# alessiodevoto/peekvit

Measured on AMD Instinct MI355X. Metric: images/sec ViT-B/16 fwd @ batch 2048, 224x224, higher is better.
Workload: dtype f16; 1 GPU; vit_b_16 forward, batch 2048/GPU, 224x224; global_batch=2048, parallelism=replicas x1 (batch-sharded, no collective), precision_mode=auto, streams=1, operands=IEEE fp16 operands, fp32 accumulate (same MFMA rate as bf16), range-guarded, range_guard_fallbacks=0

## Files before the change

peekvit_amd/_build.py:

```python
from __future__ import annotations

import glob
import os
import subprocess
import sys

HERE = os.path.dirname(os.path.abspath(__file__))
CSRC = os.path.join(HERE, "csrc")
LIB = os.path.join(HERE, "libpeekvit_hip.so")
LIB_F16 = os.path.join(HERE, "libpeekvit_hip_f16.so")
HIPCC = os.environ.get("HIPCC", "/opt/rocm/bin/hipcc")
FLAGS = ["--offload-arch=gfx950", "-O3", "-std=c++17", "-fPIC", "-Wno-unused-result"]
HEADERS = ("peekvit_hip.h", "peekvit_hip_moe.h", "peekvit_hip_ee.h", "peekvit_hip_sparse.h", "peekvit_hip_pct.h")
FILE_FLAGS = {"pv_attention.hip": ["-mllvm", "-amdgpu-mfma-vgpr-form=1"], "pv_rowops.hip": ["-fno-slp-vectorize"],
              "pv_ee.hip": ["-fno-slp-vectorize"],
              "pv_sparse.hip": ["-fno-slp-vectorize"],
              "pv_pct.hip": ["-fno-slp-vectorize"]}


def sources():
    return sorted(glob.glob(os.path.join(CSRC, "*.hip")))


def _stale() -> bool:
    if not os.path.exists(LIB) or not os.path.exists(LIB_F16):
        return True
    t = min(os.path.getmtime(LIB), os.path.getmtime(LIB_F16))
    deps = sources() + glob.glob(os.path.join(CSRC, "*.h")) + [os.path.join(os.path.dirname(HERE), "include", h) for h in HEADERS] + [os.path.abspath(__file__)]
    return any(os.path.getmtime(d) > t for d in deps)


def build(force: bool = False, verbose: bool = False) -> str:
    if not force and not _stale():
        return LIB
    procs = []
    variants = [("build", [], LIB), ("build_f16", ["-DPV_OPERAND_F16"], LIB_F16)]
    objs = {lib: [] for _, _, lib in variants}
    for sub, defs, lib in variants:
        objdir = os.path.join(HERE, sub)
        os.makedirs(objdir, exist_ok=True)
        for src in sources():
            obj = os.path.join(objdir, os.path.basename(src)[:-4] + ".o")
            objs[lib].append(obj)
            cmd = [HIPCC, *FLAGS, *FILE_FLAGS.get(os.path.basename(src), []), *defs, "-c", src, "-o", obj]
            if verbose:
                print(" ".join(cmd))
            procs.append((src, subprocess.Popen(cmd, stdout=subprocess.PIPE, stderr=subprocess.STDOUT)))
    for src, p in procs:
        out, _ = p.communicate()
        if p.returncode != 0:
# ... 35 lines not shown
```

peekvit_amd/_lib.py:

```python
from __future__ import annotations

import ctypes as C
import os
import threading

import torch

from ._build import LIB

_i64, _f32, _p, _i32 = C.c_int64, C.c_float, C.c_void_p, C.c_int32

PV_EPI_BIAS_BF16, PV_EPI_BIAS_GELU_BF16, PV_EPI_BIAS_RES_F32, PV_EPI_BIAS_POS_F32 = 0, 1, 2, 3
PV_EPI_BIAS_F32, PV_EPI_BIAS_GELU_SPLIT_BF16 = 4, 5
PV_EPI_BIAS_GELU_PAIR_BF16, PV_EPI_GELU_GRAD_BF16 = 6, 7
PV_WS_TRANSPOSE_COLSUM, PV_WS_COLSUM, PV_WS_LAYERNORM_BWD, PV_WS_GEMM_COLSUM_PARTIAL, PV_WS_GEMM_SPLITK = 1, 2, 3, 4, 5


class GemmArgs(C.Structure):
    _fields_ = [("struct_size", C.c_uint64), ("A", _p), ("W", _p), ("bias", _p), ("out", _p), ("res", _p), ("row_scale", _p), ("pos", _p),
                ("M", _i64), ("N", _i64), ("K", _i64), ("lda", _i64), ("ldw", _i64), ("ldo", _i64), ("ldr", _i64),
                ("rows_per_img_in", _i64), ("rows_per_img_out", _i64), ("row_off", _i64), ("qcols", _i64),
                ("qscale", _f32), ("epilogue", _i32),
                ("ln_gamma", _p), ("ln_beta", _p), ("ln_row_scale", _p), ("ln_out", _p), ("ln_eps", _f32),
                ("ksplit", _i32), ("colsum_partial", _p),
# ... 58 lines not shown
    "pv_residual_gate_bwd": (C.c_int, [_p, _p, _p, _p, _p, _p, _p, _f32, _f32, _p, _p, _p, _p, _i64, _i64, _i64, _p]),
    "pv_attention_varlen_bf16": (C.c_int, [_p, _p, _p, _p, _i64, _i64, _i64, _i64, _p, _p]),
    "pv_act_step": (C.c_int, [_p, _p, _p, _p, _i64, _i64, _i64, _p, _p, _p, _p, _p, _p, _i64, _p, _f32, _f32, _f32, C.c_int,
                              _p, _p, _p, _p, _p, _p, _p]),
}

SIGNATURES_MOE = {
    "pv_moe_packed_rows": (C.c_int64, [_i64, _i64]),
    "pv_moe_route_scratch_size": (C.c_int64, [_i64, _i64]),
    "pv_moe_route": (C.c_int, [_p, _i64, _i64, _i64, _p, _p, _f32, _p, _p, _i64, _p, _p, _p, _p, _p, _p, _p, _p, _i64, _p]),
    "pv_gemm_grouped_bf16": (C.c_int, [C.POINTER(GemmArgs), _p, _i64, _i64, _i64, _p, _i64, _p]),
    "pv_moe_gather_bf16": (C.c_int, [_p, _i64, _i64, _p, _p, _i64, _i64, _i64, _i64, _p, _p]),
}

SIGNATURES_EE = {
    "pv_exit_head_f32": (C.c_int, [_p, _i64, _p, _p, _f32, _p, _p, _p, _i64, _i64, _i64, _p]),
    "pv_exit_step": (C.c_int, [_p, _i64, _p, _i64, _i64, _f32, _i64, _p, _p, _i64, _p, _p, _i64, _p, _p, _p, _p]),
    "pv_gather_images_f32": (C.c_int, [_p, _i64, _p, _i64, _i64, _p, _p]),
}

SIGNATURES_SPARSE = {
    "pv_attention_varlen_w_bf16": (C.c_int, [_p, _p, _p, _p, _i64, _i64, _i64, _i64, _p, _p]),
    "pv_residual_pack_step": (C.c_int, [_p, _p, _p, _p, _i64, _i64, _i64, _p, _p, _p, _p, _f32, _f32, _p,
                                        _p, _p, _p, _p, _p, _p, _p, _p, _p, _p, _p, _f32, _p, _p]),
}

SIGNATURES_PCT = {
    "pv_arpe_embed": (C.c_int, [_p, _p, _p, _p, _p, _p, _p, _p, _p, _p, _p, _i64, _i64, _i64, _i64, _i64, _i64, _p]),
    "pv_layernorm_f32_bf16": (C.c_int, [_p, _i64, _p, _p, _p, _p, _i64, _i64, _i64, _f32, _p]),
    "pv_mean_pool_f32": (C.c_int, [_p, _p, _i64, _i64, _i64, _p]),
    "pv_pct_head_f32": (C.c_int, [_p, _p, _p, _p, _p, _p, _p, _p, _i64, _i64, _i64, _i64, _p]),
}

ABI_VERSION = 10
_lock = threading.Lock()
_libs: dict = {}

_OPERAND_DEFAULT = "bf16"
_tls = threading.local()
LIB_F16 = os.path.join(os.path.dirname(os.path.abspath(__file__)), "libpeekvit_hip_f16.so")


def current_operand() -> str:
    return getattr(_tls, "operand", _OPERAND_DEFAULT)


def set_operand(op: str) -> str:
    old = current_operand()
    _tls.operand = op
    return old


def __getattr__(name):
    if name == "OPERAND":
        return current_operand()
    raise AttributeError(f"module {__name__!r} has no attribute {name!r}")


def operand_dtype():
    import torch as _t
    return _t.float16 if current_operand() == "f16" else _t.bfloat16


class PeekvitHipError(RuntimeError):
    pass


def lib_path(operand: str = "bf16") -> str:
    return LIB_F16 if operand == "f16" else LIB


def load(operand=None):
    op = current_operand() if operand is None else operand
    lib = _libs.get(op)
    if lib is not None:
        return lib
    with _lock:
        lib = _libs.get(op)
        if lib is not None:
            return lib
        path = lib_path(op)
        if not os.path.exists(path):
            raise PeekvitHipError(
                f"{path} not found: the MI355X kernels are not built. Run `python -m peekvit_amd._build` "
                "(or __graft_entry__.build()); there is no fallback path.")
        lib = C.CDLL(path)
        for name, (res, args) in {**SIGNATURES, **SIGNATURES_MOE, **SIGNATURES_EE, **SIGNATURES_SPARSE, **SIGNATURES_PCT}.items():
            fn = getattr(lib, name)
            fn.restype, fn.argtypes = res, args
        if lib.pv_version() != ABI_VERSION:
            raise PeekvitHipError(f"{path} has ABI v{lib.pv_version()}, this package binds v{ABI_VERSION}: rebuild (python -m peekvit_amd._build)")
        if lib.pv_gemm_args_size() != C.sizeof(GemmArgs):
            raise PeekvitHipError(f"{path}: pv_gemm_args is {lib.pv_gemm_args_size()} bytes in the library, {C.sizeof(GemmArgs)} in this binding")
        if lib.pv_operand_type() != (1 if op == "f16" else 0):
            raise PeekvitHipError(f"{path} was built for a different operand type")
        _libs[op] = lib
    return lib


def check(code: int, what: str = "") -> None:
    if code != 0:
        msg = load().pv_error_string(code).decode()
        raise PeekvitHipError(f"{what}: {msg} (code {code})" if what else f"{msg} (code {code})")
```

peekvit_amd/autograph.py:

```python
from __future__ import annotations

import os
import threading
from typing import Optional

import torch
import torch.nn as nn

ENABLED = os.environ.get("PEEKVIT_AMD_AUTO_GRAPH", "1") != "0"
WARM = int(os.environ.get("PEEKVIT_AMD_AUTO_GRAPH_WARM", "4"))
MAX_GRAPHS = 4
HOST_MS_BASE, HOST_MS_PER_LAYER = 0.12, 0.115
SMALL_TFLOPS = 300.0

replays = 0
captures = 0
drops = 0

_structure_epoch = 0


def _bump(*_a, **_k):
    global _structure_epoch
    _structure_epoch += 1
    return None


try:
    import torch.nn.modules.module as _m
    _m.register_module_module_registration_hook(_bump)
    _m.register_module_parameter_registration_hook(_bump)
    _m.register_module_buffer_registration_hook(_bump)
except (ImportError, AttributeError):
    ENABLED = False


def _knobs():
    from . import engine, ops
    return (engine._STREAMS, engine.LOCAL_FALLBACK, engine.SELFCHECK_IMAGES, engine.SELFCHECK_LIMIT, engine.RANK_STRICT, engine._FUSE_LN, engine._FULLROW_LN,
            engine._FOLD_LN, engine._FUSE_RANK_NORM, engine._SMALL_M_SPLITK, engine._LAST_BLOCK_ROWS, engine._GATE_NO_MASKED, engine.FALLBACK_MODE,
            engine.RANK_REPAIR, engine.RANK_TIE_GAP, engine._FUSED_PATCH_EMBED,
            getattr(ops, "knob_epoch", 0))


def launch_bound(owner: nn.Module, batch: int) -> bool:
    try:
        D, L, S = int(owner.hidden_dim), len(owner.encoder.layers), int(owner.seq_length)
        Mh = int(getattr(owner, "mlp_dim", 4 * D))
    except (AttributeError, TypeError):
        return False
    flops = batch * L * (S * D * 3 * D * 2 + 2 * S * S * D * 2 + S * D * D * 2 + 2 * S * D * Mh * 2)
    return flops / (SMALL_TFLOPS * 1e12) < (HOST_MS_BASE + HOST_MS_PER_LAYER * L) * 1e-3


class _Entry:
    __slots__ = ("warm", "graph", "sig", "params", "mods", "calls", "dead")

    def __init__(self):
        self.warm, self.graph, self.sig, self.params, self.mods, self.calls, self.dead = 0, None, None, None, None, 0, False


_version_of = __import__("operator").attrgetter("_version")


def _signature(owner: nn.Module, ent: _Entry, st) -> tuple:
    from . import engine
    layers = getattr(getattr(owner, "encoder", None), "layers", ())
    return (_structure_epoch, engine._opt_generation, tuple(map(id, layers)), sum(map(_version_of, ent.params)), _knobs(),
            st.unsafe, st.no_fold, st.hybrid, st.mlp_hybrid, owner.training)


def _hooked(ent: _Entry) -> bool:
    import torch.nn.modules.module as _m
    if _m._global_forward_hooks or _m._global_forward_pre_hooks:
# ... 96 lines not shown
```

peekvit_amd/engine.py:

```python
from __future__ import annotations

import math
import os
import threading
import warnings
import weakref
from typing import Dict, Optional, Tuple

import torch
from torch import nn

from . import _lib, autograph, ops
import contextlib

from ._lib import (PV_EPI_BIAS_BF16, PV_EPI_BIAS_F32, PV_EPI_BIAS_GELU_BF16, PV_EPI_BIAS_GELU_SPLIT_BF16, PV_EPI_BIAS_POS_F32,
                   PV_EPI_BIAS_RES_F32, PeekvitHipError)

_MODE_DEFAULT = os.environ.get("PEEKVIT_AMD_PRECISION", "auto")
_MODES = ("auto", "bf16", "f16", "bf16x3")
if _MODE_DEFAULT not in _MODES:
    raise ValueError(f"PEEKVIT_AMD_PRECISION={_MODE_DEFAULT!r}: expected one of {_MODES}")
_lib._OPERAND_DEFAULT = "f16" if _MODE_DEFAULT == "f16" else "bf16"
_mode_tls = threading.local()

# ... 909 lines not shown
                 ln=(_f32(blk.ln_2.weight), _f32(blk.ln_2.bias), eps, h2, row_scale) if fuse2 else None)
        ln2_done = fuse2
    else:
        ln2_done = _residual_gemm(att, bf16_weight(mha.out_proj.weight), _f32(mha.out_proj.bias), x1.view(R, D), x.view(R, D), R,
                                  ln=(_f32(blk.ln_2.weight), _f32(blk.ln_2.bias), eps, h2))
    if mlp_hyb:
        _mlp_half_split(blk, x1, out, R, eps, row_scale)
        return out
    if not ln2_done:
        ops.layernorm_bf16(x1, _f32(blk.ln_2.weight), _f32(blk.ln_2.bias), eps, h2, row_scale)
    _act_gemm(h2, bf16_weight(blk.mlp.fc1.weight), _f32(blk.mlp.fc1.bias), g, R, gelu=True)
    fuse_next = next_ln is not None and _ln_fusable(D, M) and next_ln.normalized_shape == (D,)
    hn = workspace.get("h", (R, D), _lib.operand_dtype(), dev) if fuse_next else None
    rowsq = None
    if next_ranks and not fuse_next and _FUSE_RANK_NORM and ops.gemm_tile_rows(R, D, M, PV_EPI_BIAS_RES_F32) == 256:
        rowsq = workspace.get("rowsq", ((D + 255) // 256, R), torch.float32, dev)
    if fuse_next or rowsq is not None:
        ops.gemm(g, bf16_weight(blk.mlp.fc2.weight), _f32(blk.mlp.fc2.bias), out.view(R, D), PV_EPI_BIAS_RES_F32, M=R,
                 res=x1.view(R, D), rowsq_out=rowsq,
                 ln=(_f32(next_ln.weight), _f32(next_ln.bias), next_ln.eps, hn, None) if fuse_next else None)
    else:
        want = next_ln is not None and next_ln.normalized_shape == (D,)
        hn = workspace.get("h", (R, D), _lib.operand_dtype(), dev) if want else None
        fuse_next = _residual_gemm(g, bf16_weight(blk.mlp.fc2.weight), _f32(blk.mlp.fc2.bias), out.view(R, D), x1.view(R, D), R,
                                   ln=(_f32(next_ln.weight), _f32(next_ln.bias), next_ln.eps, hn) if want else None)
    if fuse_next:
        out._pv_ln = (hn, _ln_key(next_ln))
    if rowsq is not None:
        out._pv_rowsq = (rowsq, _tver(out))
    return out


_LAST_BLOCK_ROWS = os.environ.get("PEEKVIT_AMD_LAST_BLOCK_ROWS", "1") != "0"
_GATE_LN1 = os.environ.get("PEEKVIT_AMD_GATE_LN1", "1") != "0"
_GATE_NO_MASKED = os.environ.get("PEEKVIT_AMD_GATE_MASKED", "0") != "1"


def rows_only_ok(blk: nn.Module) -> bool:
    import torch.nn.modules.module as _m
    if not _LAST_BLOCK_ROWS or _mode() == "bf16x3" or layer_is_hybrid() or layer_mlp_is_hybrid():
        return False
    own = ("_forward_hooks", "_forward_pre_hooks", "_backward_hooks", "_backward_pre_hooks")
    glob = ("_global_forward_hooks", "_global_forward_pre_hooks", "_global_backward_hooks", "_global_backward_pre_hooks")
    return not any(getattr(blk, n, None) for n in own) and not any(getattr(_m, n, None) for n in glob)


def block_forward_rows(blk: nn.Module, x: torch.Tensor, eps: float, nq: int, row_scale: Optional[torch.Tensor] = None,
                       h1: Optional[torch.Tensor] = None) -> torch.Tensor:
    if x.dtype != torch.float32:
        x = x.float()
    fold_in, handoff = getattr(x, "_pv_fold", None), getattr(x, "_pv_ln", None)
    if fold_in is not None and fold_in[3] != _tver(x):
        fold_in = None
    if not x.is_contiguous():
        x, fold_in, handoff = x.contiguous(), None, None
    if row_scale is not None:
        fold_in, handoff = None, None
    B, S, D = x.shape
    mha = blk.self_attention.self_attention
    H = mha.num_heads
    dh = D // H
    M = blk.mlp.fc1.out_features
    dev, R, Rq, od = x.device, B * S, B * nq, _lib.operand_dtype()
    _check_ln_range(blk.ln_1)
    _check_ln_range(blk.ln_2)
    g1, b1 = _f32(blk.ln_1.weight), _f32(blk.ln_1.bias)

    kv = workspace.get("qkv", (R, 2 * D), od, dev)
    if fold_in is not None and fold_in[2] == _ln_key(blk.ln_1) and fold_in[0].shape == (R, D):
        wg, c1, c2 = _fold_weights(mha.in_proj_weight, mha.in_proj_bias, blk.ln_1)
        stat = ops.rowstat_finalize(fold_in[1], D, blk.ln_1.eps, workspace.get("fold_stat", (R, 2), torch.float32, dev))
        ops.gemm(fold_in[0], wg[D:], None, kv, PV_EPI_BIAS_BF16, M=R, fold=(stat, c1[D:], c2[D:]))
    else:
        if h1 is not None and h1.shape == (R, D):
            h = h1
        elif handoff is not None and handoff[1] == _ln_key(blk.ln_1) and handoff[0].shape == (R, D):
            h = handoff[0]
        else:
            h = workspace.get("h", (R, D), od, dev)
            ops.layernorm_bf16(x, g1, b1, eps, h, row_scale)
        ops.gemm(h, bf16_weight(mha.in_proj_weight)[D:], _f32(mha.in_proj_bias)[D:], kv, PV_EPI_BIAS_BF16, M=R)

    xq = workspace.get("rows_x", (B, nq, D), torch.float32, dev)
    xq.copy_(x[:, :nq])
    xq = xq.view(Rq, D)
    rsq = None
    if row_scale is not None:
        rsq = workspace.get("rows_rs", (B, nq), torch.float32, dev)
        rsq.copy_(row_scale.view(B, S)[:, :nq])
    hq = workspace.get("rows_h", (Rq, D), od, dev)
    ops.layernorm_bf16(xq, g1, b1, eps, hq, rsq)
    qb = workspace.get("rows_q", (Rq, D), od, dev)
    ops.gemm(hq, bf16_weight(mha.in_proj_weight)[:D], _f32(mha.in_proj_bias)[:D], qb, PV_EPI_BIAS_BF16, M=Rq, qcols=D, qscale=float(dh) ** -0.5)
    att = workspace.get("rows_att", (Rq, D), od, dev)
    ops.attention_rows(qb, kv, att, B, S, nq, H, dh)
    x1 = workspace.get("rows_x1", (Rq, D), torch.float32, dev)
    if rsq is None:
        _residual_gemm(att, bf16_weight(mha.out_proj.weight), _f32(mha.out_proj.bias), x1, xq, Rq)
    else:
        ops.gemm(att, bf16_weight(mha.out_proj.weight), _f32(mha.out_proj.bias), x1, PV_EPI_BIAS_RES_F32, M=Rq, res=xq, row_scale=rsq)
    ops.layernorm_bf16(x1, _f32(blk.ln_2.weight), _f32(blk.ln_2.bias), eps, hq, rsq)
    g = workspace.get("rows_g", (Rq, M), od, dev)
    ops.gemm(hq, bf16_weight(blk.mlp.fc1.weight), _f32(blk.mlp.fc1.bias), g, PV_EPI_BIAS_GELU_BF16, M=Rq)
    out = torch.empty((B, nq, D), dtype=torch.float32, device=dev)
    _residual_gemm(g, bf16_weight(blk.mlp.fc2.weight), _f32(blk.mlp.fc2.bias), out.view(Rq, D), x1, Rq)
    return out


def _block_forward_x3(blk: nn.Module, x: torch.Tensor, eps: float, row_scale: Optional[torch.Tensor]) -> torch.Tensor:
    x = x.float() if x.dtype != torch.float32 else x
    x = x if x.is_contiguous() else x.contiguous()
    B, S, D = x.shape
    mha = blk.self_attention.self_attention
    H = mha.num_heads
    dh = D // H
    M = blk.mlp.fc1.out_features
    dev, R = x.device, B * S
    h3 = workspace.get("h3", (R, 3 * D), _lib.operand_dtype(), dev)
    qkv32 = workspace.get("qkv32", (R, 3 * D), torch.float32, dev)
    att3 = workspace.get("att3", (R, 3 * D), _lib.operand_dtype(), dev)
    g3 = workspace.get("g3", (R, 3 * M), _lib.operand_dtype(), dev)
    x1 = workspace.get("x1", (B, S, D), torch.float32, dev)
    out = torch.empty_like(x)
    ops.layernorm_split(x, _f32(blk.ln_1.weight), _f32(blk.ln_1.bias), eps, h3, row_scale)
    ops.gemm(h3, bf16x3_weight(mha.in_proj_weight), _f32(mha.in_proj_bias), qkv32, PV_EPI_BIAS_F32, M=R, qcols=D, qscale=float(dh) ** -0.5)
    ops.attention_f32(qkv32, att3, B, S, H, dh)
    ops.gemm(att3, bf16x3_weight(mha.out_proj.weight), _f32(mha.out_proj.bias), x1.view(R, D), PV_EPI_BIAS_RES_F32, M=R,
             res=x.view(R, D), row_scale=row_scale)
# ... 722 lines not shown
```

peekvit_amd/ops.py:

```python
from __future__ import annotations

import ctypes as C
from typing import Optional

import torch

from . import _lib
from ._lib import GemmArgs, check

launch_count = 0


class KernelTimer:

    def __init__(self):
        self.records = []

    def __enter__(self):
        global _timer
        _timer = self
        return self

    def __exit__(self, *exc):
        global _timer
# ... 232 lines not shown
    N = b.shape[1]
    assert b.shape[0] == K and part.shape == (max(ksplit, 1), M, N) and part.is_contiguous()
    args = GemmArgs(A=a.data_ptr(), W=b.data_ptr(), bias=0, out=part.data_ptr(), res=0, row_scale=0, pos=0, M=M, N=N, K=K,
                    lda=a.stride(0), ldw=b.stride(0), ldo=N, ldr=0, rows_per_img_in=0, rows_per_img_out=0, row_off=0, qcols=0,
                    qscale=1.0, epilogue=_lib.PV_EPI_BIAS_F32, ln_gamma=0, ln_beta=0, ln_row_scale=0, ln_out=0, ln_eps=0.0,
                    ksplit=int(ksplit))
    with _timed("pv_gemm_tn_bf16" + tag, a.device, 2.0 * M * N * K, 2.0 * K * (M + N) + 4.0 * max(ksplit, 1) * M * N):
        check(_lib.load().pv_gemm_tn_bf16(C.byref(args), _stream(a)), "pv_gemm_tn_bf16")
    _count()
    return part


def attention(qkv: torch.Tensor, out: torch.Tensor, B: int, S: int, H: int, dh: int, lse: Optional[torch.Tensor] = None):
    with _timed("pv_attention_bf16", qkv.device, 4.0 * B * H * S * S * dh, 8.0 * B * S * H * dh):
        if lse is None:
            check(_lib.load().pv_attention_bf16(_ptr(qkv), _ptr(out), B, S, H, dh, _attn_flag(qkv.device), _stream(qkv)), "pv_attention_bf16")
        else:
            _chk(lse, torch.float32, "lse")
            if lse.numel() != B * H * S:
                raise _lib.PeekvitHipError("attention: lse must hold B * H * S values")
            check(_lib.load().pv_attention_lse_bf16(_ptr(qkv), _ptr(out), _ptr(lse), B, S, H, dh, _attn_flag(qkv.device), _stream(qkv)), "pv_attention_lse_bf16")
    _count()
    return out


def attention_bwd_lse_ok(S: int, dh: int) -> bool:
    return attention_bwd_lse_supported(S, dh) and S >= 145


def attention_bwd_lse_supported(S: int, dh: int) -> bool:
    return dh in (48, 64) and 129 <= S <= 208


def attention_rows(q: torch.Tensor, kv: torch.Tensor, out: torch.Tensor, B: int, S: int, nq: int, H: int, dh: int):
    for t, name in ((q, "q"), (kv, "kv"), (out, "out")):
        if not (t.is_cuda and t.dtype == _lib.operand_dtype() and t.dim() == 2 and t.stride(1) == 1):
            raise _lib.PeekvitHipError(f"attention_rows: {name} must be a 2-D GPU tensor of the operand type with unit column stride")
    if q.shape[0] != B * nq or out.shape[0] != B * nq or kv.shape[0] != B * S or kv.shape[1] < 2 * H * dh:
        raise _lib.PeekvitHipError("attention_rows: shape mismatch")
    with _timed("pv_attention_rows_bf16", q.device, 4.0 * B * H * nq * S * dh, 4.0 * B * S * H * dh + 4.0 * B * nq * H * dh):
        check(_lib.load().pv_attention_rows_bf16(_ptr(q), q.stride(0), _ptr(kv), kv.stride(0), _ptr(out), out.stride(0),
                                                 B, S, nq, H, dh, _attn_flag(q.device), _stream(q)), "pv_attention_rows_bf16")
    _count()
    return out


def attention_rows_bwd(q, kv, out, dout, dq, dkv, B: int, S: int, H: int, dh: int, qscale: float):
    for t, name in ((q, "q"), (kv, "kv"), (out, "out"), (dout, "dout"), (dq, "dq"), (dkv, "dkv")):
        if not (t.is_cuda and t.dtype == _lib.operand_dtype() and t.dim() == 2 and t.stride(1) == 1):
            raise _lib.PeekvitHipError(f"attention_rows_bwd: {name} must be a 2-D GPU tensor of the operand type with unit column stride")
    if any(t.shape[0] != B for t in (q, out, dout, dq)) or kv.shape[0] != B * S or dkv.shape[0] != B * S:
        raise _lib.PeekvitHipError("attention_rows_bwd: shape mismatch")
    with _timed("pv_attention_rows_bwd_bf16", q.device, 10.0 * B * H * S * dh, 2.0 * 3 * 2 * B * S * H * dh):
        check(_lib.load().pv_attention_rows_bwd_bf16(_ptr(q), q.stride(0), _ptr(kv), kv.stride(0), _ptr(out), out.stride(0), _ptr(dout), dout.stride(0),
                                                     _ptr(dq), dq.stride(0), _ptr(dkv), dkv.stride(0), B, S, 1, H, dh, float(qscale), _stream(q)),
              "pv_attention_rows_bwd_bf16")
    _count()
    return dq, dkv


def cls_pool(x: torch.Tensor, gamma, beta, eps: float, num_cls: int) -> torch.Tensor:
    B, S, D = x.shape
    pooled = torch.empty((B, D), dtype=torch.float32, device=x.device)
    with _timed("pv_cls_pool", x.device, 0.0, 0.0):
        check(_lib.load().pv_cls_pool(_ptr(x), _ptr(gamma), _ptr(beta), _ptr(pooled), B, S, D, num_cls, float(eps),
                                      _stream(x)), "pv_cls_pool")
    _count()
    return pooled


def head(pooled: torch.Tensor, w: torch.Tensor, b) -> torch.Tensor:
    B, D = pooled.shape
    Cn = w.shape[0]
    logits = torch.empty((B, Cn), dtype=torch.float32, device=pooled.device)
    with _timed("pv_head_f32", pooled.device, 2.0 * B * D * Cn, 0.0):
# ... 576 lines not shown
```

Before: 27530 images/sec.

## Fold K/V projection into CLS-row attention to skip full-token KV GEMM

For the final block where only a few query rows (CLS) are needed, the K and V projection of all tokens is no longer materialised. Instead, each query is folded into the key weights (u = q·Wk), scores are computed directly against the raw or LayerNorm-folded tokens, a softmax-weighted token average is accumulated, and the value projection is then applied once per query row. This replaces an R x 2D x D GEMM with work that scales with the number of query rows times heads, at the cost of three new kernels, fp32 scratch buffers, and hi/lo split MFMA for precision.

```diff
diff --git a/include/peekvit_hip_cls.h b/include/peekvit_hip_cls.h
--- /dev/null
+++ b/include/peekvit_hip_cls.h
@@ -0,0 +1,27 @@
+#ifndef PEEKVIT_HIP_CLS_H
+#define PEEKVIT_HIP_CLS_H
+
+#include "peekvit_hip.h"
+
+#ifdef __cplusplus
+extern "C" {
+#endif
+
+#define PV_CLS_MAX_D 768
+#define PV_CLS_MAX_ROWS 32
+
+int pv_cls_attention_built(int64_t S, int64_t D, int64_t H, int64_t dh, int64_t nq);
+
+int pv_cls_query_fold_bf16(const uint16_t* q, int64_t ldq, const uint16_t* wk, int64_t ldw, const float* c1k, const float* c2k, float* u,
+                           float* cd, int64_t rows, int64_t H, int64_t dh, void* stream);
+
+int pv_cls_token_pass_bf16(const uint16_t* tok, int64_t ldt, const float* stat, const float* u, const float* cd, float* a, float* m,
+                           int64_t B, int64_t S, int64_t D, int64_t nr, uint32_t* range_flag, void* stream);
+
+int pv_cls_value_fold_bf16(const float* a, const float* m, const uint16_t* wv, int64_t ldw, const float* c1v, const float* c2v,
+                           uint16_t* att, int64_t ldo, int64_t rows, int64_t H, int64_t dh, void* stream);
+
+#ifdef __cplusplus
+}
+#endif
+#endif
diff --git a/peekvit_amd/_build.py b/peekvit_amd/_build.py
--- a/peekvit_amd/_build.py
+++ b/peekvit_amd/_build.py
@@ -11,11 +11,12 @@
 LIB_F16 = os.path.join(HERE, "libpeekvit_hip_f16.so")
 HIPCC = os.environ.get("HIPCC", "/opt/rocm/bin/hipcc")
 FLAGS = ["--offload-arch=gfx950", "-O3", "-std=c++17", "-fPIC", "-Wno-unused-result"]
-HEADERS = ("peekvit_hip.h", "peekvit_hip_moe.h", "peekvit_hip_ee.h", "peekvit_hip_sparse.h", "peekvit_hip_pct.h")
+HEADERS = ("peekvit_hip.h", "peekvit_hip_moe.h", "peekvit_hip_ee.h", "peekvit_hip_sparse.h", "peekvit_hip_pct.h", "peekvit_hip_cls.h")
 FILE_FLAGS = {"pv_attention.hip": ["-mllvm", "-amdgpu-mfma-vgpr-form=1"], "pv_rowops.hip": ["-fno-slp-vectorize"],
               "pv_ee.hip": ["-fno-slp-vectorize"],
               "pv_sparse.hip": ["-fno-slp-vectorize"],
-              "pv_pct.hip": ["-fno-slp-vectorize"]}
+              "pv_pct.hip": ["-fno-slp-vectorize"],
+              "pv_cls_attention.hip": ["-fno-slp-vectorize"]}
 
 
 def sources():
diff --git a/peekvit_amd/_lib.py b/peekvit_amd/_lib.py
--- a/peekvit_amd/_lib.py
+++ b/peekvit_amd/_lib.py
@@ -114,6 +114,13 @@
     "pv_pct_head_f32": (C.c_int, [_p, _p, _p, _p, _p, _p, _p, _p, _i64, _i64, _i64, _i64, _p]),
 }
 
+SIGNATURES_CLS = {
+    "pv_cls_attention_built": (C.c_int, [_i64, _i64, _i64, _i64, _i64]),
+    "pv_cls_query_fold_bf16": (C.c_int, [_p, _i64, _p, _i64, _p, _p, _p, _p, _i64, _i64, _i64, _p]),
+    "pv_cls_token_pass_bf16": (C.c_int, [_p, _i64, _p, _p, _p, _p, _p, _i64, _i64, _i64, _i64, _p, _p]),
+    "pv_cls_value_fold_bf16": (C.c_int, [_p, _p, _p, _i64, _p, _p, _p, _i64, _i64, _i64, _i64, _p]),
+}
+
 ABI_VERSION = 10
 _lock = threading.Lock()
 _libs: dict = {}
@@ -167,7 +174,7 @@
                 f"{path} not found: the MI355X kernels are not built. Run `python -m peekvit_amd._build` "
                 "(or __graft_entry__.build()); there is no fallback path.")
         lib = C.CDLL(path)
-        for name, (res, args) in {**SIGNATURES, **SIGNATURES_MOE, **SIGNATURES_EE, **SIGNATURES_SPARSE, **SIGNATURES_PCT}.items():
+        for name, (res, args) in {**SIGNATURES, **SIGNATURES_MOE, **SIGNATURES_EE, **SIGNATURES_SPARSE, **SIGNATURES_PCT, **SIGNATURES_CLS}.items():
             fn = getattr(lib, name)
             fn.restype, fn.argtypes = res, args
         if lib.pv_version() != ABI_VERSION:
diff --git a/peekvit_amd/autograph.py b/peekvit_amd/autograph.py
--- a/peekvit_amd/autograph.py
+++ b/peekvit_amd/autograph.py
@@ -39,7 +39,7 @@
     from . import engine, ops
     return (engine._STREAMS, engine.LOCAL_FALLBACK, engine.SELFCHECK_IMAGES, engine.SELFCHECK_LIMIT, engine.RANK_STRICT, engine._FUSE_LN, engine._FULLROW_LN,
             engine._FOLD_LN, engine._FUSE_RANK_NORM, engine._SMALL_M_SPLITK, engine._LAST_BLOCK_ROWS, engine._GATE_NO_MASKED, engine.FALLBACK_MODE,
-            engine.RANK_REPAIR, engine.RANK_TIE_GAP, engine._FUSED_PATCH_EMBED,
+            engine.RANK_REPAIR, engine.RANK_TIE_GAP, engine._FUSED_PATCH_EMBED, engine._CLS_ATTENTION,
             getattr(ops, "knob_epoch", 0))
 
 
diff --git a/peekvit_amd/csrc/pv_cls_attention.hip b/peekvit_amd/csrc/pv_cls_attention.hip
--- /dev/null
+++ b/peekvit_amd/csrc/pv_cls_attention.hip
@@ -0,0 +1,385 @@
+#include "pv_common.h"
+#include "../../include/peekvit_hip_cls.h"
+
+#define PV_CLS_QR 8
+__global__ __launch_bounds__(128) void pv_cls_qfold_kernel(const uint16_t* __restrict__ q, int64_t ldq, const uint16_t* __restrict__ wk, int64_t ldw,
+                                                           const float* __restrict__ c1k, const float* __restrict__ c2k, float* __restrict__ u,
+                                                           float* __restrict__ cd, int64_t rows, int H, int dh) {
+    __shared__ __attribute__((aligned(16))) float qs[64][PV_CLS_QR];
+    const int t = threadIdx.x;
+    const int h = (int)(blockIdx.x % H);
+    const int64_t r0 = (int64_t)(blockIdx.x / H) * PV_CLS_QR;
+    const int D = H * dh;
+    for (int idx = t; idx < PV_CLS_QR * dh; idx += 128) {
+        const int r = idx / dh, j = idx - r * dh;
+        qs[j][r] = r0 + r < rows ? pv_bf2f(q[(r0 + r) * ldq + h * dh + j]) : 0.f;
+    }
+    __syncthreads();
+    const uint16_t* wrow = wk + (int64_t)h * dh * ldw;
+    for (int kd = t; kd < (D >> 1); kd += 128) {
+        float acc[PV_CLS_QR][2];
+#pragma unroll
+        for (int r = 0; r < PV_CLS_QR; ++r) acc[r][0] = acc[r][1] = 0.f;
+#pragma unroll 4
+        for (int j = 0; j < dh; ++j) {
+            const uint32_t wd = *reinterpret_cast<const uint32_t*>(wrow + (int64_t)j * ldw + 2 * kd);
+            const float lo = pv_unpack_lo(wd), hi = pv_unpack_hi(wd);
+            const f32x4 qa = *reinterpret_cast<const f32x4*>(&qs[j][0]), qb = *reinterpret_cast<const f32x4*>(&qs[j][4]);
+#pragma unroll
+            for (int r = 0; r < 4; ++r) {
+                acc[r][0] += qa[r] * lo;
+                acc[r][1] += qa[r] * hi;
+                acc[r + 4][0] += qb[r] * lo;
+                acc[r + 4][1] += qb[r] * hi;
+            }
+        }
+#pragma unroll
+        for (int r = 0; r < PV_CLS_QR; ++r)
+            if (r0 + r < rows) {
+                float* p = u + ((r0 + r) * H + h) * (int64_t)D + 2 * kd;
+                p[0] = acc[r][0];
+                p[1] = acc[r][1];
+            }
+    }
+    if (t < PV_CLS_QR && r0 + t < rows) {
+        float c = 0.f, d = 0.f;
+        for (int j = 0; j < dh; ++j) {
+            if (c1k != nullptr) c += c1k[h * dh + j] * qs[j][t];
+            if (c2k != nullptr) d += c2k[h * dh + j] * qs[j][t];
+        }
+        cd[((r0 + t) * H + h) * 2] = c;
+        cd[((r0 + t) * H + h) * 2 + 1] = d;
+    }
+}
+
+#define PV_CLS_CHUNK 16
+__device__ __forceinline__ float pv_cls_row16_max(float v) {
+    v = fmaxf(v, __builtin_bit_cast(float, __builtin_amdgcn_update_dpp(0, __builtin_bit_cast(int, v), 0xB1, 0xf, 0xf, true)));
+    v = fmaxf(v, __builtin_bit_cast(float, __builtin_amdgcn_update_dpp(0, __builtin_bit_cast(int, v), 0x4E, 0xf, 0xf, true)));
+    v = fmaxf(v, __builtin_bit_cast(float, __builtin_amdgcn_update_dpp(0, __builtin_bit_cast(int, v), 0x141, 0xf, 0xf, true)));
+    v = fmaxf(v, __builtin_bit_cast(float, __builtin_amdgcn_update_dpp(0, __builtin_bit_cast(int, v), 0x140, 0xf, 0xf, true)));
+    return v;
+}
+
+template <int RW, int KS>
+__global__ __launch_bounds__(256) void pv_cls_tokens_kernel(const uint16_t* __restrict__ tok, int64_t ldt, const float* __restrict__ stat,
+                                                            const float* __restrict__ u, const float* __restrict__ cd, float* __restrict__ a,
+                                                            float* __restrict__ mo, int S, int D, int NR, uint32_t* flag) {
+    constexpr int NRT = (4 * RW + 15) / 16;
+    constexpr int NRP = 4 * RW;
+    constexpr int LDT = KS * 128 + 8;
+    __shared__ __attribute__((aligned(16))) uint16_t tokS[PV_CLS_CHUNK * LDT];
+    __shared__ f32x4 partS[4 * NRT * 64];
+    __shared__ __attribute__((aligned(16))) float pS[PV_CLS_CHUNK * NRP];
+    __shared__ float scaleS[NRP];
+
+    const int t = threadIdx.x, lane = t & 63, w = t >> 6;
+    const int64_t img = blockIdx.x;
+    const int nks = D >> 5, dq8 = D >> 3, dw = D >> 1;
+    const int l15 = lane & 15, lg = lane >> 4;
+
+    u32x4 uh[NRT][KS], ul[NRT][KS];
+#pragma unroll
+    for (int tt = 0; tt < NRT; ++tt)
+#pragma unroll
+        for (int i = 0; i < KS; ++i) {
+            const int ks = w + 4 * i, row = tt * 16 + l15;
+            f32x4 x0 = {0.f, 0.f, 0.f, 0.f}, x1 = x0;
+            if (ks < nks && row < NR) {
+                const float* p = u + (img * NR + row) * (int64_t)D + ks * 32 + 8 * lg;
+                x0 = *reinterpret_cast<const f32x4*>(p);
+                x1 = *reinterpret_cast<const f32x4*>(p + 4);
+            }
+            const PvHiLo s0 = pv_split2(x0[0], x0[1]), s1 = pv_split2(x0[2], x0[3]), s2 = pv_split2(x1[0], x1[1]), s3 = pv_split2(x1[2], x1[3]);
+            uh[tt][i] = u32x4{s0.hi, s1.hi, s2.hi, s3.hi};
+            ul[tt][i] = u32x4{s0.lo, s1.lo, s2.lo, s3.lo};
+        }
+
+    float cr[4], dr[4], mrun[4], lrun[4], mac[4];
+#pragma unroll
+    for (int r = 0; r < 4; ++r) {
+        const int row = w * 16 + 4 * lg + r;
+        const bool have = w < NRT && row < NR;
+        cr[r] = have ? cd[(img * NR + row) * 2] : 0.f;
+        dr[r] = have ? cd[(img * NR + row) * 2 + 1] : 0.f;
+        mrun[r] = -INFINITY;
+        lrun[r] = 0.f;
+        mac[r] = 0.f;
+    }
+
+    int prow[KS], pcol[KS];
+#pragma unroll
+    for (int i = 0; i < KS; ++i) {
+        const int p = t + 256 * i;
+        prow[i] = p / dq8;
+        pcol[i] = (p - prow[i] * dq8) * 8;
+    }
+    const uint16_t* timg = tok + img * S * ldt;
+    u32x4 pre[KS];
+#pragma unroll
+    for (int i = 0; i < KS; ++i) {
+        pre[i] = u32x4{0u, 0u, 0u, 0u};
+        if (prow[i] < PV_CLS_CHUNK) {
+            const int s = prow[i] < S ? prow[i] : S - 1;
+            pre[i] = *reinterpret_cast<const u32x4*>(timg + (int64_t)s * ldt + pcol[i]);
+        }
+    }
+
+    float acc[RW][KS][2];
+#pragma unroll
+    for (int i = 0; i < RW; ++i)
+#pragma unroll
+        for (int j = 0; j < KS; ++j) acc[i][j][0] = acc[i][j][1] = 0.f;
+    int cdw[KS];
+#pragma unroll
+    for (int j = 0; j < KS; ++j) cdw[j] = 64 * j + lane < dw ? 64 * j + lane : dw - 1;
+
+    for (int s0 = 0; s0 < S; s0 += PV_CLS_CHUNK) {
+#pragma unroll
+        for (int i = 0; i < KS; ++i)
+            if (prow[i] < PV_CLS_CHUNK) *reinterpret_cast<u32x4*>(&tokS[prow[i] * LDT + pcol[i]]) = pre[i];
+        __syncthreads();
+        if (s0 + PV_CLS_CHUNK < S) {
+#pragma unroll
+            for (int i = 0; i < KS; ++i)
+                if (prow[i] < PV_CLS_CHUNK) {
+                    const int s = s0 + PV_CLS_CHUNK + prow[i] < S ? s0 + PV_CLS_CHUNK + prow[i] : S - 1;
+                    pre[i] = *reinterpret_cast<const u32x4*>(timg + (int64_t)s * ldt + pcol[i]);
+                }
+        }
+        f32x4 sc[NRT];
+#pragma unroll
+        for (int tt = 0; tt < NRT; ++tt) sc[tt] = f32x4{0.f, 0.f, 0.f, 0.f};
+#pragma unroll
+        for (int i = 0; i < KS; ++i) {
+            const int ks = w + 4 * i;
+            if (ks < nks) {
+                const u32x4 b = *reinterpret_cast<const u32x4*>(&tokS[l15 * LDT + ks * 32 + 8 * lg]);
+#pragma unroll
+                for (int tt = 0; tt < NRT; ++tt) {
+                    sc[tt] = PV_MFMA_16x16x32(uh[tt][i], b, sc[tt], 0, 0, 0);
+                    sc[tt] = PV_MFMA_16x16x32(ul[tt][i], b, sc[tt], 0, 0, 0);
+                }
+            }
+        }
+#pragma unroll
+        for (int tt = 0; tt < NRT; ++tt) partS[(w * NRT + tt) * 64 + lane] = sc[tt];
+        __syncthreads();
+        if (w < NRT) {
+            const f32x4 d4 = (partS[(0 * NRT + w) * 64 + lane] + partS[(1 * NRT + w) * 64 + lane]) +
+                             (partS[(2 * NRT + w) * 64 + lane] + partS[(3 * NRT + w) * 64 + lane]);
+            const int s = s0 + l15;
+            const bool valid = s < S;
+            float mu = 0.f, rs = 1.f;
+            if (stat != nullptr) {
+                const int64_t si = img * S + (valid ? s : S - 1);
+                mu = stat[2 * si];
+                rs = stat[2 * si + 1];
+            }
+#pragma unroll
+            for (int r = 0; r < 4; ++r) {
+                const int row = w * 16 + 4 * lg + r;
+                const float x = valid ? rs * (d4[r] - mu * cr[r]) + dr[r] : -INFINITY;
+                const float mn = fmaxf(mrun[r], pv_cls_row16_max(x));
+                const float scl = __expf(mrun[r] - mn);
+                const float p = valid ? __expf(x - mn) : 0.f;
+                const float wgt = p * rs;
+                lrun[r] = lrun[r] * scl + p;
+                mac[r] = mac[r] * scl + wgt * mu;
+                mrun[r] = mn;
+                if (row < NRP) {
+                    const int slot = (row & 3) * RW + (row >> 2);
+                    pS[l15 * NRP + slot] = wgt;
+                    if (l15 == 0) scaleS[slot] = scl;
+                }
+            }
+        }
+        __syncthreads();
+        float scl[RW];
+#pragma unroll
+        for (int i = 0; i < RW; ++i) scl[i] = scaleS[w * RW + i];
+#pragma unroll
+        for (int i = 0; i < RW; ++i)
+#pragma unroll
+            for (int j = 0; j < KS; ++j) {
+                acc[i][j][0] *= scl[i];
+                acc[i][j][1] *= scl[i];
+            }
+        const int ns = S - s0 < PV_CLS_CHUNK ? S - s0 : PV_CLS_CHUNK;
+        const uint32_t* tokW = reinterpret_cast<const uint32_t*>(tokS);
+#pragma unroll 4
+        for (int s = 0; s < ns; ++s) {
+            float wg[RW];
+#pragma unroll
+            for (int i = 0; i < RW; ++i) wg[i] = pS[s * NRP + w * RW + i];
+#pragma unroll
+            for (int j = 0; j < KS; ++j) {
+                const uint32_t v = tokW[s * (LDT / 2) + cdw[j]];
+                const float lo = pv_unpack_lo(v), hi = pv_unpack_hi(v);
+#pragma unroll
+                for (int i = 0; i < RW; ++i) {
+                    acc[i][j][0] += wg[i] * lo;
+                    acc[i][j][1] += wg[i] * hi;
+                }
+            }
+        }
+        __syncthreads();
+    }
+
+    if (w < NRT) {
+#pragma unroll
+        for (int r = 0; r < 4; ++r) {
+            const int row = w * 16 + 4 * lg + r;
+            const float l = pv_row16_sum(lrun[r]), ms = pv_row16_sum(mac[r]);
+            if (row < NR) pv_score_guard(mrun[r], flag);
+            if (l15 == 0 && row < NRP) {
+                const float inv = 1.0f / l;
+                scaleS[(row & 3) * RW + (row >> 2)] = inv;
+                if (row < NR) mo[img * NR + row] = ms * inv;
+            }
+        }
+    }
+    __syncthreads();
+#pragma unroll
+    for (int i = 0; i < RW; ++i) {
+        const int row = w + 4 * i;
+        if (row >= NR) continue;
+        const float inv = scaleS[w * RW + i];
+        float* arow = a + (img * NR + row) * (int64_t)D;
+#pragma unroll
+        for (int j = 0; j < KS; ++j)
+            if (64 * j + lane < dw) {
+                arow[2 * (64 * j + lane)] = acc[i][j][0] * inv;
+                arow[2 * (64 * j + lane) + 1] = acc[i][j][1] * inv;
+            }
+    }
+}
+
+#define PV_CLS_VR 4
+__global__ __launch_bounds__(256) void pv_cls_vfold_kernel(const float* __restrict__ a, const float* __restrict__ m, const uint16_t* __restrict__ wv,
+                                                           int64_t ldw, const float* __restrict__ c1v, const float* __restrict__ c2v,
+                                                           uint16_t* __restrict__ att, int64_t ldo, int64_t rows, int H, int dh) {
+    const int lane = threadIdx.x & 63, w = threadIdx.x >> 6;
+    const int h = (int)(blockIdx.x % H);
+    const int64_t r0 = (int64_t)(blockIdx.x / H) * PV_CLS_VR;
+    const int D = H * dh, dq8 = D >> 3;
+    float av[PV_CLS_VR][2][8];
+#pragma unroll
+    for (int r = 0; r < PV_CLS_VR; ++r)
+#pragma unroll
+        for (int c = 0; c < 2; ++c) {
+            const int ck = lane + 64 * c;
+            f32x4 x0 = {0.f, 0.f, 0.f, 0.f}, x1 = x0;
+            if (ck < dq8 && r0 + r < rows) {
+                const float* p = a + ((r0 + r) * H + h) * (int64_t)D + ck * 8;
+                x0 = *reinterpret_cast<const f32x4*>(p);
+                x1 = *reinterpret_cast<const f32x4*>(p + 4);
+            }
+#pragma unroll
+            for (int e = 0; e < 4; ++e) {
+                av[r][c][e] = x0[e];
+                av[r][c][e + 4] = x1[e];
+            }
+        }
+    for (int jj = w; jj < dh; jj += 8) {
+        const int n = h * dh + jj;
+        float s[2 * PV_CLS_VR];
+#pragma unroll
+        for (int i = 0; i < 2 * PV_CLS_VR; ++i) s[i] = 0.f;
+#pragma unroll
+        for (int c = 0; c < 2; ++c) {
+            const int ck = lane + 64 * c < dq8 ? lane + 64 * c : dq8 - 1;
+            const u32x4 wd0 = *reinterpret_cast<const u32x4*>(wv + (int64_t)n * ldw + ck * 8);
+            const u32x4 wd1 = *reinterpret_cast<const u32x4*>(wv + (int64_t)(n + 4) * ldw + ck * 8);
+#pragma unroll
+            for (int e = 0; e < 4; ++e) {
+                const float lo0 = pv_unpack_lo(wd0[e]), hi0 = pv_unpack_hi(wd0[e]), lo1 = pv_unpack_lo(wd1[e]), hi1 = pv_unpack_hi(wd1[e]);
+#pragma unroll
+                for (int r = 0; r < PV_CLS_VR; ++r) {
+                    s[r] += lo0 * av[r][c][2 * e] + hi0 * av[r][c][2 * e + 1];
+                    s[PV_CLS_VR + r] += lo1 * av[r][c][2 * e] + hi1 * av[r][c][2 * e + 1];
+                }
+            }
+        }
+        const float tot = pv_reduce8_rows(s, lane);
+        const int i = lane >> 3, nn = n + 4 * (i >> 2);
+        const int64_t row = r0 + (i & 3);
+        if ((lane & 7) == 0 && row < rows) {
+            float o = tot;
+            if (c1v != nullptr) o -= m[row * H + h] * c1v[nn];
+            if (c2v != nullptr) o += c2v[nn];
+            att[row * ldo + nn] = pv_f2bf(o);
+        }
+    }
+}
+
+static bool pv_cls_dims_ok(int64_t D, int64_t H, int64_t dh) {
+    return (dh == 32 || dh == 48 || dh == 64) && H >= 1 && D == H * dh && D % 64 == 0 && D <= PV_CLS_MAX_D;
+}
+
+extern "C" int pv_cls_attention_built(int64_t S, int64_t D, int64_t H, int64_t dh, int64_t nq) {
+    return S >= 1 && S < 0x40000000LL && D >= 1 && H >= 1 && dh >= 1 && nq >= 1 && pv_cls_dims_ok(D, H, dh) && nq * H <= PV_CLS_MAX_ROWS ? 1 : 0;
+}
+
+extern "C" int pv_cls_query_fold_bf16(const uint16_t* q, int64_t ldq, const uint16_t* wk, int64_t ldw, const float* c1k, const float* c2k,
+                                      float* u, float* cd, int64_t rows, int64_t H, int64_t dh, void* stream) {
+    if (!q || !wk || !u || !cd || rows <= 0 || H <= 0 || dh <= 0) return PV_ERR_INVALID_ARG;
+    if (((uintptr_t)q & 15) || ((uintptr_t)wk & 15) || ((uintptr_t)u & 15) || ((uintptr_t)cd & 7) || ((uintptr_t)c1k & 3) || ((uintptr_t)c2k & 3))
+        return PV_ERR_INVALID_ARG;
+    if (H > PV_CLS_MAX_D || dh > PV_CLS_MAX_D) return PV_ERR_UNSUPPORTED;
+    const int64_t D = H * dh;
+    if ((ldq & 7) || (ldw & 7) || ldq < D || ldw < D) return PV_ERR_INVALID_ARG;
+    if (!pv_cls_dims_ok(D, H, dh)) return PV_ERR_UNSUPPORTED;
+    const int64_t blocks = (rows + PV_CLS_QR - 1) / PV_CLS_QR * H;
+    if (blocks > 0x7fffffffLL) return PV_ERR_UNSUPPORTED;
+    PV_LAUNCH(pv_cls_qfold_kernel, dim3((unsigned)blocks), dim3(128), 0, (hipStream_t)stream, q, ldq, wk, ldw, c1k, c2k, u, cd, rows, (int)H, (int)dh);
+    return pv_check_launch();
+}
+
+template <int RW, int KS>
+static int pv_launch_cls_tokens(const uint16_t* tok, int64_t ldt, const float* stat, const float* u, const float* cd, float* a, float* m, int64_t B,
+                                int S, int D, int nr, uint32_t* flag, hipStream_t stream) {
+    PV_LAUNCH((pv_cls_tokens_kernel<RW, KS>), dim3((unsigned)B), dim3(256), 0, stream, tok, ldt, stat, u, cd, a, m, S, D, nr, flag);
+    return pv_check_launch();
+}
+
+template <int KS>
+static int pv_dispatch_cls_tokens(const uint16_t* tok, int64_t ldt, const float* stat, const float* u, const float* cd, float* a, float* m,
+                                  int64_t B, int S, int D, int nr, uint32_t* flag, hipStream_t stream) {
+    const int rw = (nr + 3) / 4;
+#define PV_CLS_TOK(N) return pv_launch_cls_tokens<N, KS>(tok, ldt, stat, u, cd, a, m, B, S, D, nr, flag, stream)
+    if (rw <= 1) PV_CLS_TOK(1);
+    if (rw == 2) PV_CLS_TOK(2);
+    if (rw == 3) PV_CLS_TOK(3);
+    if (rw == 4) PV_CLS_TOK(4);
+    if (rw <= 6) PV_CLS_TOK(6);
+    PV_CLS_TOK(8);
+#undef PV_CLS_TOK
+}
+
+extern "C" int pv_cls_token_pass_bf16(const uint16_t* tok, int64_t ldt, const float* stat, const float* u, const float* cd, float* a, float* m,
+                                      int64_t B, int64_t S, int64_t D, int64_t nr, uint32_t* range_flag, void* stream) {
+    if (!tok || !u || !cd || !a || !m || B <= 0 || S <= 0 || D <= 0 || nr <= 0 || ((uintptr_t)range_flag & 3)) return PV_ERR_INVALID_ARG;
+    if (((uintptr_t)tok & 15) || ((uintptr_t)u & 15) || ((uintptr_t)a & 15) || ((uintptr_t)stat & 7) || ((uintptr_t)cd & 7) || ((uintptr_t)m & 3))
+        return PV_ERR_INVALID_ARG;
+    if ((ldt & 7) || ldt < D) return PV_ERR_INVALID_ARG;
+    if (D % 64 != 0 || D > PV_CLS_MAX_D || nr > PV_CLS_MAX_ROWS || B > 0x7fffffffLL || S >= 0x40000000LL) return PV_ERR_UNSUPPORTED;
+    hipStream_t s = (hipStream_t)stream;
+    if (D <= 384) return pv_dispatch_cls_tokens<3>(tok, ldt, stat, u, cd, a, m, B, (int)S, (int)D, (int)nr, range_flag, s);
+    return pv_dispatch_cls_tokens<6>(tok, ldt, stat, u, cd, a, m, B, (int)S, (int)D, (int)nr, range_flag, s);
+}
+
+extern "C" int pv_cls_value_fold_bf16(const float* a, const float* m, const uint16_t* wv, int64_t ldw, const float* c1v, const float* c2v,
+                                      uint16_t* att, int64_t ldo, int64_t rows, int64_t H, int64_t dh, void* stream) {
+    if (!a || !wv || !att || rows <= 0 || H <= 0 || dh <= 0 || (c1v && !m)) return PV_ERR_INVALID_ARG;
+    if (((uintptr_t)a & 15) || ((uintptr_t)wv & 15) || ((uintptr_t)att & 15) || ((uintptr_t)m & 3) || ((uintptr_t)c1v & 3) || ((uintptr_t)c2v & 3))
+        return PV_ERR_INVALID_ARG;
+    if (H > PV_CLS_MAX_D || dh > PV_CLS_MAX_D) return PV_ERR_UNSUPPORTED;
+    const int64_t D = H * dh;
+    if ((ldw & 7) || ldw < D || ldo < D) return PV_ERR_INVALID_ARG;
+    if (!pv_cls_dims_ok(D, H, dh)) return PV_ERR_UNSUPPORTED;
+    const int64_t blocks = (rows + PV_CLS_VR - 1) / PV_CLS_VR * H;
+    if (blocks > 0x7fffffffLL) return PV_ERR_UNSUPPORTED;
+    PV_LAUNCH(pv_cls_vfold_kernel, dim3((unsigned)blocks), dim3(256), 0, (hipStream_t)stream, a, m, wv, ldw, c1v, c2v, att, ldo, rows, (int)H, (int)dh);
+    return pv_check_launch();
+}
diff --git a/peekvit_amd/engine.py b/peekvit_amd/engine.py
--- a/peekvit_amd/engine.py
+++ b/peekvit_amd/engine.py
@@ -965,6 +965,7 @@
 
 
 _LAST_BLOCK_ROWS = os.environ.get("PEEKVIT_AMD_LAST_BLOCK_ROWS", "1") != "0"
+_CLS_ATTENTION = os.environ.get("PEEKVIT_AMD_CLS_ATTENTION", "1") != "0"
 _GATE_LN1 = os.environ.get("PEEKVIT_AMD_GATE_LN1", "1") != "0"
 _GATE_NO_MASKED = os.environ.get("PEEKVIT_AMD_GATE_MASKED", "0") != "1"
 
@@ -999,11 +1000,16 @@
     _check_ln_range(blk.ln_2)
     g1, b1 = _f32(blk.ln_1.weight), _f32(blk.ln_1.bias)
 
-    kv = workspace.get("qkv", (R, 2 * D), od, dev)
+    cls = _CLS_ATTENTION and row_scale is None and h1 is None and ops.attention_rows_tokens_ok(S, D, H, dh, nq)
+    kv, tok = None, None
     if fold_in is not None and fold_in[2] == _ln_key(blk.ln_1) and fold_in[0].shape == (R, D):
         wg, c1, c2 = _fold_weights(mha.in_proj_weight, mha.in_proj_bias, blk.ln_1)
         stat = ops.rowstat_finalize(fold_in[1], D, blk.ln_1.eps, workspace.get("fold_stat", (R, 2), torch.float32, dev))
-        ops.gemm(fold_in[0], wg[D:], None, kv, PV_EPI_BIAS_BF16, M=R, fold=(stat, c1[D:], c2[D:]))
+        if cls:
+            tok = dict(tokens=fold_in[0], stat=stat, w=wg[D:], c1=c1[D:], c2=c2[D:])
+        else:
+            kv = workspace.get("qkv", (R, 2 * D), od, dev)
+            ops.gemm(fold_in[0], wg[D:], None, kv, PV_EPI_BIAS_BF16, M=R, fold=(stat, c1[D:], c2[D:]))
     else:
         if h1 is not None and h1.shape == (R, D):
             h = h1
@@ -1012,7 +1018,11 @@
         else:
             h = workspace.get("h", (R, D), od, dev)
             ops.layernorm_bf16(x, g1, b1, eps, h, row_scale)
-        ops.gemm(h, bf16_weight(mha.in_proj_weight)[D:], _f32(mha.in_proj_bias)[D:], kv, PV_EPI_BIAS_BF16, M=R)
+        if cls:
+            tok = dict(tokens=h, w=bf16_weight(mha.in_proj_weight)[D:], c2=_f32(mha.in_proj_bias)[D:])
+        else:
+            kv = workspace.get("qkv", (R, 2 * D), od, dev)
+            ops.gemm(h, bf16_weight(mha.in_proj_weight)[D:], _f32(mha.in_proj_bias)[D:], kv, PV_EPI_BIAS_BF16, M=R)
 
     xq = workspace.get("rows_x", (B, nq, D), torch.float32, dev)
     xq.copy_(x[:, :nq])
@@ -1026,7 +1036,12 @@
     qb = workspace.get("rows_q", (Rq, D), od, dev)
     ops.gemm(hq, bf16_weight(mha.in_proj_weight)[:D], _f32(mha.in_proj_bias)[:D], qb, PV_EPI_BIAS_BF16, M=Rq, qcols=D, qscale=float(dh) ** -0.5)
     att = workspace.get("rows_att", (Rq, D), od, dev)
-    ops.attention_rows(qb, kv, att, B, S, nq, H, dh)
+    if tok is not None:
+        tok["work"] = (workspace.get("cls_u", (Rq * H, D), torch.float32, dev), workspace.get("cls_cd", (Rq * H, 2), torch.float32, dev),
+                       workspace.get("cls_a", (Rq * H, D), torch.float32, dev), workspace.get("cls_m", (Rq * H,), torch.float32, dev))
+        ops.attention_rows(qb, None, att, B, S, nq, H, dh, **tok)
+    else:
+        ops.attention_rows(qb, kv, att, B, S, nq, H, dh)
     x1 = workspace.get("rows_x1", (Rq, D), torch.float32, dev)
     if rsq is None:
         _residual_gemm(att, bf16_weight(mha.out_proj.weight), _f32(mha.out_proj.bias), x1, xq, Rq)
diff --git a/peekvit_amd/ops.py b/peekvit_amd/ops.py
--- a/peekvit_amd/ops.py
+++ b/peekvit_amd/ops.py
@@ -288,15 +288,70 @@
     return dh in (48, 64) and 129 <= S <= 208
 
 
-def attention_rows(q: torch.Tensor, kv: torch.Tensor, out: torch.Tensor, B: int, S: int, nq: int, H: int, dh: int):
-    for t, name in ((q, "q"), (kv, "kv"), (out, "out")):
+_cls_built: dict = {}
+
+
+def attention_rows_tokens_ok(S: int, D: int, H: int, dh: int, nq: int) -> bool:
+    key = (int(S), int(D), int(H), int(dh), int(nq), _lib.current_operand())
+    ok = _cls_built.get(key)
+    if ok is None:
+        ok = _cls_built[key] = bool(_lib.load().pv_cls_attention_built(*key[:5]))
+    return ok
+
+
+def attention_rows(q: torch.Tensor, kv: Optional[torch.Tensor], out: torch.Tensor, B: int, S: int, nq: int, H: int, dh: int, *,
+                   tokens: Optional[torch.Tensor] = None, stat: Optional[torch.Tensor] = None, w: Optional[torch.Tensor] = None,
+                   c1: Optional[torch.Tensor] = None, c2: Optional[torch.Tensor] = None, work=None):
+    D = H * dh
+    if tokens is None:
+        for t, name in ((q, "q"), (kv, "kv"), (out, "out")):
+            if not (t is not None and t.is_cuda and t.dtype == _lib.operand_dtype() and t.dim() == 2 and t.stride(1) == 1):
+                raise _lib.PeekvitHipError(f"attention_rows: {name} must be a 2-D GPU tensor of the operand type with unit column stride")
+        if q.shape[0] != B * nq or out.shape[0] != B * nq or kv.shape[0] != B * S or kv.shape[1] < 2 * H * dh:
+            raise _lib.PeekvitHipError("attention_rows: shape mismatch")
+        with _timed("pv_attention_rows_bf16", q.device, 4.0 * B * H * nq * S * dh, 4.0 * B * S * H * dh + 4.0 * B * nq * H * dh):
+            check(_lib.load().pv_attention_rows_bf16(_ptr(q), q.stride(0), _ptr(kv), kv.stride(0), _ptr(out), out.stride(0),
+                                                     B, S, nq, H, dh, _attn_flag(q.device), _stream(q)), "pv_attention_rows_bf16")
+        _count()
+        return out
+    if kv is not None or w is None:
+        raise _lib.PeekvitHipError("attention_rows: the token form takes tokens and w, and no kv")
+    for t, name in ((q, "q"), (tokens, "tokens"), (out, "out"), (w, "w")):
         if not (t.is_cuda and t.dtype == _lib.operand_dtype() and t.dim() == 2 and t.stride(1) == 1):
             raise _lib.PeekvitHipError(f"attention_rows: {name} must be a 2-D GPU tensor of the operand type with unit column stride")
-    if q.shape[0] != B * nq or out.shape[0] != B * nq or kv.shape[0] != B * S or kv.shape[1] < 2 * H * dh:
+    if (q.shape[0] != B * nq or out.shape[0] != B * nq or q.shape[1] < D or out.shape[1] < D or tokens.shape[0] != B * S or tokens.shape[1] < D
+            or w.shape[0] != 2 * D or w.shape[1] != D):
         raise _lib.PeekvitHipError("attention_rows: shape mismatch")
-    with _timed("pv_attention_rows_bf16", q.device, 4.0 * B * H * nq * S * dh, 4.0 * B * S * H * dh + 4.0 * B * nq * H * dh):
-        check(_lib.load().pv_attention_rows_bf16(_ptr(q), q.stride(0), _ptr(kv), kv.stride(0), _ptr(out), out.stride(0),
-                                                 B, S, nq, H, dh, _attn_flag(q.device), _stream(q)), "pv_attention_rows_bf16")
+    if (stat is None) != (c1 is None):
+        raise _lib.PeekvitHipError("attention_rows: row statistics and c1 come together (the LayerNorm-folded form) or not at all")
+    for t, name, n in ((stat, "stat", 2 * B * S), (c1, "c1", 2 * D), (c2, "c2", 2 * D)):
+        if t is not None and (_chk(t, torch.float32, name).numel() != n or t.device != q.device):
+            raise _lib.PeekvitHipError(f"attention_rows: {name} must hold {n} fp32 values on the queries' device")
+    if not attention_rows_tokens_ok(S, D, H, dh, nq):
+        raise _lib.PeekvitHipError(f"attention_rows: the token form is not built for S={S}, D={D}, H={H}, dh={dh}, nq={nq} (ask attention_rows_tokens_ok first)")
+    Rq, nr, dev = B * nq, nq * H, q.device
+    if work is None:
+        work = (torch.empty((Rq * H, D), dtype=torch.float32, device=dev), torch.empty((Rq * H, 2), dtype=torch.float32, device=dev),
+                torch.empty((Rq * H, D), dtype=torch.float32, device=dev), torch.empty((Rq * H,), dtype=torch.float32, device=dev))
+    u, cd, a, m = work
+    for t, name, n in ((u, "u", Rq * H * D), (cd, "cd", Rq * H * 2), (a, "a", Rq * H * D), (m, "m", Rq * H)):
+        if _chk(t, torch.float32, "work." + name).numel() != n or t.device != dev:
+            raise _lib.PeekvitHipError(f"attention_rows: work.{name} must hold {n} fp32 values on the queries' device")
+    lib = _lib.load()
+    wk, wv = w[:D], w[D:]
+    with _timed("pv_cls_query_fold_bf16", dev, 2.0 * Rq * D * D, 2.0 * Rq * D + 2.0 * D * D + 4.0 * Rq * H * D):
+        check(lib.pv_cls_query_fold_bf16(_ptr(q), q.stride(0), _ptr(wk), w.stride(0), _ptr(c1), _ptr(c2), _ptr(u), _ptr(cd), Rq, H, dh, _stream(q)),
+              "pv_cls_query_fold_bf16")
+    _count()
+    with _timed("pv_attention_rows_bf16", dev, 4.0 * B * S * D * nr, 2.0 * B * S * D + (8.0 * B * S if stat is not None else 0.0) + 8.0 * Rq * H * D):
+        check(lib.pv_cls_token_pass_bf16(_ptr(tokens), tokens.stride(0), _ptr(stat), _ptr(u), _ptr(cd), _ptr(a), _ptr(m), B, S, D, nr,
+                                         _attn_flag(dev), _stream(q)), "pv_cls_token_pass_bf16")
+    _count()
+    c1v = None if c1 is None else c1[D:]
+    c2v = None if c2 is None else c2[D:]
+    with _timed("pv_cls_value_fold_bf16", dev, 2.0 * Rq * D * D, 4.0 * Rq * H * D + 2.0 * D * D + 2.0 * Rq * D):
+        check(lib.pv_cls_value_fold_bf16(_ptr(a), _ptr(m), _ptr(wv), w.stride(0), _ptr(c1v), _ptr(c2v), _ptr(out), out.stride(0), Rq, H, dh, _stream(q)),
+              "pv_cls_value_fold_bf16")
     _count()
     return out
 
```

Result: no change. 27780 images/sec, median of 6 (+0.9%).
